# luicalrob/Triangulation-in-Deformable-Scenes

Measured on AMD Instinct MI355X. Metric: LM iterations/sec + ms/iter at 100k corr × 2 views; 1/2/4/8-GPU scaling, higher is better.
Workload: dtype f64

## Files before the change

### triangulation-in-deformable-scenes_amd/csrc/kernels.h

```cpp
#pragma once
#include <hip/hip_runtime.h>

#include <cstdint>
#include <vector>

namespace deftri {

constexpr int64_t kHeavyChunks = 16;

struct DevProblem {
    int32_t P = 0, Q = 0, S = 0, C = 0, R = 0, D = 0, E = 0, NR = 0;
    double *points = nullptr, *scales = nullptr, *tg = nullptr;
    double *points_bak = nullptr, *scales_bak = nullptr, *tg_bak = nullptr;
    float *cam_kb8 = nullptr;
    double *cam_pose = nullptr, *cam_R = nullptr;
    int32_t *rep_point = nullptr, *rep_cam = nullptr;
    double *rep_obs = nullptr, *rep_info = nullptr;
    double huber_delta = 0;
    int32_t *dep_point = nullptr, *dep_scale = nullptr, *dep_cam = nullptr;
    double *dep_meas = nullptr, *dep_info = nullptr;
    int32_t *arap_pts = nullptr, *arap_pair = nullptr, *arap_rot = nullptr;
    double *arap_w = nullptr, *rot = nullptr, *pair_area = nullptr, *pair_info = nullptr;
    double *Jrep = nullptr, *Wrep = nullptr, *Erep = nullptr, *chi_rep = nullptr;
    double *Jdep = nullptr, *Wdep = nullptr, *Edep = nullptr, *chi_dep = nullptr;
    double *Jarap = nullptr, *Warap = nullptr, *Earap = nullptr, *chi_arap = nullptr;
    int64_t jarap_ld = 0;
    double *tg_pre = nullptr;
    const int *gate_lin = nullptr, *gate_trial = nullptr;
    double *lin_part = nullptr;
    int64_t n_arap_sum = 0;
};

struct FrontDev {
    const int32_t *m, *s, *parent, *nchild, *child0, *child1, *direct, *rhs_bnd, *panel_off;
    const int64_t *arena_off, *vec_off, *rows_off, *bmap_off, *inv_off;
    const int32_t *rows, *bmap;
};

struct LevelDev {
    int64_t ea_off[2]; int32_t nea[2];
    struct Step { int64_t diag_off; int32_t ndiag; int64_t trsm_off; int32_t ntrsm; int64_t upd_off; int32_t nupd; int32_t k0, kA, kmax, inner, stream, wait_side; double upd_flops; int32_t ntail, ndiag_tail; };
    std::vector<Step> steps;
    int64_t fwd_off; int32_t nfwd;
    struct SolveStep { int64_t off; int32_t n; };
    std::vector<SolveStep> fsteps, bsteps;
// ... 142 lines not shown
```

### triangulation-in-deformable-scenes_amd/csrc/kernels.hip

```cpp
#include <hip/hip_runtime.h>

#include <algorithm>
#include <atomic>
#include <cstdint>
#include <cstdlib>

#include "device_math.h"
#include "diag_panel.h"
#include "kernels.h"
#include "symbolic.h"
#include "ticket.h"

namespace deftri {
namespace dev {

#define TID (blockIdx.x * blockDim.x + threadIdx.x)

__device__ __forceinline__ void huber_rho(double delta, double e2, double &rho0, double &rho1) {
#pragma clang fp contract(off)
    if (delta <= 0) { rho0 = e2; rho1 = 1.0; return; }
    double dsqr = delta * delta;
    if (e2 <= dsqr) { rho0 = e2; rho1 = 1.0; }
    else { double se = sqrt(e2); rho0 = 2 * se * delta - dsqr; rho1 = delta / se; }
}

__device__ __forceinline__ double lin_rep_edge(int e, int R, const int32_t *__restrict__ rp, const int32_t *__restrict__ rc,
// ... 240 lines not shown
    if (k > 0) {
        const double delta = 1e-9;
        double uu[6] = {0, 0, 0, 0, 0, 0};
        uu[(k - 1) >> 1] = (k & 1) ? delta : -delta;
        X = se3_mul(se3_exp(uu), T);
    }
    double *o = pre + 12 * (int64_t)t;
    quat_to_mat(X.r, o);
    o[9] = X.t[0]; o[10] = X.t[1]; o[11] = X.t[2];
}
__global__ void k_arap_pre(int Q, const double *__restrict__ tg, double *__restrict__ pre, const int *gate) {
    if (gate && !*gate) return;
    arap_pre_one(TID, Q, tg, pre);
}

template <int MODE>
__device__ __forceinline__ double lin_arap_edge(int e, int E_, const int32_t *__restrict__ apts, const int32_t *__restrict__ apair,
                           const int32_t *__restrict__ arot, const double *__restrict__ aw,
                           const double *__restrict__ rot, const double *__restrict__ parea,
                           const double *__restrict__ pinfo, const double *__restrict__ points,
                           const double *__restrict__ tg, const double *__restrict__ tg_pre,
                           double *__restrict__ J, double *__restrict__ W,
                           double *__restrict__ E, double *__restrict__ chi, int want_jac, int analytic,
                           int64_t jld) {
    if (e >= E_) return 0.0;
    const int32_t *v = apts + 4 * (int64_t)e;
    double P[4][3];
#pragma unroll
    for (int k = 0; k < 4; k++) {
        const double *pp = points + 3 * (int64_t)v[k];
        P[k][0] = pp[0]; P[k][1] = pp[1]; P[k][2] = pp[2];
    }
    int q = apair[e];
    SE3 T = se3_load(tg + 7 * q);
    const double *Ri = rot + 9 * (int64_t)arot[2 * (int64_t)e];
    const double *Rj = rot + 9 * (int64_t)arot[2 * (int64_t)e + 1];
    double w = aw[e], om = pinfo[q];
    const AreaDiv area = area_div(parea[q]);
    double err = arap_err(P[0], P[1], P[2], P[3], T, Ri, Rj, w, area);
// ... 25 lines not shown
            Jv[0 + k] = -rv[k] - 2.0 * g[k];
            Jv[3 + k] = qv[k] + rg[k];
            Jv[6 + k] = rv[k] - 2.0 * g[k];
            Jv[9 + k] = -qv[k] + rg[k];
        }
        Jv[12] = 2.0 * (u[1] * g[2] - u[2] * g[1]);
        Jv[13] = 2.0 * (u[2] * g[0] - u[0] * g[2]);
        Jv[14] = 2.0 * (u[0] * g[1] - u[1] * g[0]);
        Jv[15] = -4.0 * g[0]; Jv[16] = -4.0 * g[1]; Jv[17] = -4.0 * g[2];
    } else if (MODE == 2) {
#pragma clang fp contract(off)
        auto jst = [&](int k, double v) {
            if (jld) J[k * jld + e] = v;
            else J[18 * (int64_t)e + k] = v;
        };
        bool negz = false;
#pragma unroll
        for (int a = 0; a < 4; a++)
#pragma unroll
            for (int k = 0; k < 3; k++) negz |= __double_as_longlong(P[a][k]) == (long long)0x8000000000000000ull;
        if (negz) {
            const double delta = 1e-9, scalar = 1.0 / (2 * delta);
            const double *X = tg_pre + 12 * kArapPre * (int64_t)q;
#pragma unroll
            for (int vi = 0; vi < 4; vi++)
#pragma unroll 1
                for (int dd = 0; dd < 3; dd++) {
                    double Pp[4][3], Pm[4][3];
#pragma unroll
                    for (int a = 0; a < 4; a++)
#pragma unroll
                        for (int k = 0; k < 3; k++) {
                            const double d = (a == vi && k == dd) ? delta : 0.0;
                            Pp[a][k] = P[a][k] + d;
                            Pm[a][k] = P[a][k] - d;
                        }
                    const double ep = arap_err_rt(Pp[0], Pp[1], Pp[2], Pp[3], X, X + 9, Ri, Rj, w, area);
                    const double em = arap_err_rt(Pm[0], Pm[1], Pm[2], Pm[3], X, X + 9, Ri, Rj, w, area);
                    jst(3 * vi + dd, scalar * (ep - em));
                }
#pragma unroll 1
            for (int dd = 0; dd < 6; dd++) {
                const double *Xp = X + 12 * (1 + 2 * dd), *Xm = Xp + 12;
                const double ep = arap_err_rt(P[0], P[1], P[2], P[3], Xp, Xp + 9, Ri, Rj, w, area);
                const double em = arap_err_rt(P[0], P[1], P[2], P[3], Xm, Xm + 9, Ri, Rj, w, area);
                jst(12 + dd, scalar * (ep - em));
            }
        } else {
            const double delta = 1e-9, scalar = 1.0 / (2 * delta);
            const double *X = tg_pre + 12 * kArapPre * (int64_t)q;
            double Rg[12];
#pragma unroll
            for (int k = 0; k < 12; k++) Rg[k] = X[k];
            ArapBase bm;
            arap_base(P[0], P[1], P[2], P[3], Rg, Rg + 9, Ri, Rj, area, bm);
            const double fgm = arap_fg(bm.f, bm.g);
#pragma unroll 1
            for (int dd = 0; dd < 6; dd++) {
                const double *Xp = X + 12 * (1 + 2 * dd), *Xm = Xp + 12;
                double dp[3], dm[3];
#pragma unroll
                for (int k = 0; k < 3; k++) {
                    dp[k] = ((arap_mrow(Xp + 3 * k, P[1]) - Xp[9 + k]) - P[0][k]) + ((arap_mrow(Xp + 3 * k, P[3]) - Xp[9 + k]) - P[2][k]);
                    dm[k] = ((arap_mrow(Xm + 3 * k, P[1]) - Xm[9 + k]) - P[0][k]) + ((arap_mrow(Xm + 3 * k, P[3]) - Xm[9 + k]) - P[2][k]);
                }
                jst(12 + dd, scalar * (arap_sum_fg(dp, fgm, w) - arap_sum_fg(dm, fgm, w)));
            }
            auto point = [&](auto VI_, auto DD_) {
                constexpr int VI = decltype(VI_)::value, DD = decltype(DD_)::value;
                const double ep = arap_pert<VI, DD>(bm, P, P[VI][DD] + delta, Rg, Rg + 9, Ri, Rj, w, area);
                const double em = arap_pert<VI, DD>(bm, P, P[VI][DD] - delta, Rg, Rg + 9, Ri, Rj, w, area);
                jst(3 * VI + DD, scalar * (ep - em));
            };
            using std::integral_constant;
            point(integral_constant<int, 0>{}, integral_constant<int, 0>{});
            point(integral_constant<int, 0>{}, integral_constant<int, 1>{});
            point(integral_constant<int, 0>{}, integral_constant<int, 2>{});
            point(integral_constant<int, 1>{}, integral_constant<int, 0>{});
            point(integral_constant<int, 1>{}, integral_constant<int, 1>{});
            point(integral_constant<int, 1>{}, integral_constant<int, 2>{});
            point(integral_constant<int, 2>{}, integral_constant<int, 0>{});
            point(integral_constant<int, 2>{}, integral_constant<int, 1>{});
            point(integral_constant<int, 2>{}, integral_constant<int, 2>{});
            point(integral_constant<int, 3>{}, integral_constant<int, 0>{});
            point(integral_constant<int, 3>{}, integral_constant<int, 1>{});
            point(integral_constant<int, 3>{}, integral_constant<int, 2>{});
        }
    } else {
#pragma clang fp contract(off)
        const double delta = 1e-9, scalar = 1.0 / (2 * delta);
        const double *X = tg_pre + 12 * kArapPre * (int64_t)q;
        double Rg[12];
#pragma unroll
        for (int k = 0; k < 12; k++) Rg[k] = X[k];
#pragma unroll
        for (int vi = 0; vi < 4; vi++)
#pragma unroll 1
            for (int dd = 0; dd < 3; dd++) {
                double Pp[4][3], Pm[4][3];
#pragma unroll
                for (int a = 0; a < 4; a++)
// ... 13 lines not shown
        for (int dd = 0; dd < 6; dd++) {
            const double *Xp = X + 12 * (1 + 2 * dd), *Xm = Xp + 12;
            double ep = arap_err_rt(P[0], P[1], P[2], P[3], Xp, Xp + 9, Ri, Rj, w, area);
            double em = arap_err_rt(P[0], P[1], P[2], P[3], Xm, Xm + 9, Ri, Rj, w, area);
            Jv[12 + dd] = scalar * (ep - em);
        }
    }
    if (MODE != 2) {
        if (jld) {
#pragma unroll
            for (int k = 0; k < 18; k++) J[k * jld + e] = Jv[k];
        } else {
            for (int k = 0; k < 18; k++) J[18 * (int64_t)e + k] = Jv[k];
        }
    }
    W[e] = om;
    E[e] = err;
    return c2;
}

__device__ __forceinline__ double block128_sum(double v) {
    __shared__ double r2[2];
    for (int off = 32; off > 0; off >>= 1) v += __shfl_xor(v, off, 64);
    if ((threadIdx.x & 63) == 0) r2[threadIdx.x >> 6] = v;
    __syncthreads();
    return r2[0] + r2[1];
}

__global__ void k_lin_rep(int R, const int32_t *__restrict__ rp, const int32_t *__restrict__ rc,
                          const double *__restrict__ obs, const double *__restrict__ info, double hdelta,
// ... 11 lines not shown
                          const double *__restrict__ scales, const double *__restrict__ cam_pose,
                          const double *__restrict__ cam_R, double *__restrict__ J, double *__restrict__ W,
                          double *__restrict__ E, double *__restrict__ chi, int want_jac, int analytic, const int *gate) {
    if (gate && !*gate) return;
    lin_dep_edge(TID, D, dpt, dsc, dcam, meas, info, points, scales, cam_pose, cam_R, J, W, E, chi, want_jac, analytic);
}

template <int MODE>
__global__ void __launch_bounds__(128) __attribute__((amdgpu_waves_per_eu(MODE == 2 ? 2 : 1, 8))) k_lin_arap(int E_, const int32_t *__restrict__ apts, const int32_t *__restrict__ apair,
                           const int32_t *__restrict__ arot, const double *__restrict__ aw,
                           const double *__restrict__ rot, const double *__restrict__ parea,
                           const double *__restrict__ pinfo, const double *__restrict__ points,
                           const double *__restrict__ tg, const double *__restrict__ tg_pre,
                           double *__restrict__ J, double *__restrict__ W,
                           double *__restrict__ E, double *__restrict__ chi, int want_jac, int analytic,
                           int64_t jld, const int *gate, double *__restrict__ lpart, int64_t nsum) {
    if (gate && !*gate) return;
    const double c = lin_arap_edge<MODE>(TID, E_, apts, apair, arot, aw, rot, parea, pinfo, points, tg, tg_pre, J, W, E,
                                         lpart ? nullptr : chi, want_jac, analytic, jld);
    if (lpart && (int64_t)blockIdx.x * 128 < nsum) {
        const double v = block128_sum(TID < nsum ? c : 0.0);
        if (threadIdx.x == 0) lpart[blockIdx.x] = v;
    }
}

__global__ void __launch_bounds__(128) k_lin_pts(const DevProblem P, int nbr, int nbd, int want_jac, int analytic) {
    if (P.gate_lin && !*P.gate_lin) return;
    const int b = blockIdx.x, t = threadIdx.x;
    double c = 0.0;
    if (b < nbr)
        c = lin_rep_edge(b * 128 + t, P.R, P.rep_point, P.rep_cam, P.rep_obs, P.rep_info, P.huber_delta, P.points,
                         P.cam_pose, P.cam_R, P.cam_kb8, P.Jrep, P.Wrep, P.Erep, P.lin_part ? nullptr : P.chi_rep,
                         want_jac);
    else if (b < nbr + nbd)
        c = lin_dep_edge((b - nbr) * 128 + t, P.D, P.dep_point, P.dep_scale, P.dep_cam, P.dep_meas, P.dep_info, P.points,
                         P.scales, P.cam_pose, P.cam_R, P.Jdep, P.Wdep, P.Edep, P.lin_part ? nullptr : P.chi_dep,
                         want_jac, analytic);
// ... 1566 lines not shown
    return v;
}

void launch_linearize(const DevProblem &P, hipStream_t st, bool want_jac, bool analytic) {
    const bool pre = want_jac && !analytic && P.E > 0;
    const int nbr = P.R > 0 ? (int)nb(P.R, 128) : 0, nbd = P.D > 0 ? (int)nb(P.D, 128) : 0;
    const int nbp = pre ? (int)nb((int64_t)P.Q * dev::kArapPre, 128) : 0;
    LAUNCH("lin_pts", dev::k_lin_pts, dim3(nbr + nbd + nbp), dim3(128), st, P, nbr, nbd, want_jac ? 1 : 0,
           analytic ? 1 : 0);
    if (P.E > 0)
        LAUNCH("lin_arap", (!want_jac ? dev::k_lin_arap<0> : analytic ? dev::k_lin_arap<1> : arap_j_full() ? dev::k_lin_arap<3> : dev::k_lin_arap<2>),
                           dim3(nb(P.E, 128)), dim3(128), st, P.E, P.arap_pts, P.arap_pair,
                           P.arap_rot, P.arap_w, P.rot, P.pair_area, P.pair_info, P.points, P.tg,
                           pre ? P.tg_pre : nullptr, P.Jarap, P.Warap, P.Earap, P.chi_arap, want_jac ? 1 : 0,
                           analytic ? 1 : 0, P.jarap_ld, P.gate_lin, P.lin_part ? P.lin_part + nbr + nbd : nullptr,
                           P.n_arap_sum);
}

void launch_assemble(const DevProblem &P, const DevPlan &L, hipStream_t st) {
    dev::EdgeJ ej{P.Jrep, P.Wrep, P.Erep, P.Jdep, P.Wdep, P.Edep, P.Jarap, P.Warap, P.Earap};
    if (L.nhchunks > 0)
        LAUNCH("hchunk", dev::k_hchunk, dim3(nb(L.nhchunks, 64)), dim3(64), st, L.nhchunks, L.hcontrib,
                           L.hchunk_begin, L.hchunk_len, ej, L.hpart);
    if (L.nblocks > 0)
        LAUNCH("hfinal", dev::k_hfinal, dim3(nb(L.nblocks, 128)), dim3(128), st, L.nblocks,
                           L.hblk_chunk_begin, L.blk_val_off, L.blk_rows, L.blk_cols, L.hpart, L.hval);
    if (L.nheavy_h > 0) {
        LAUNCH("hfinal_heavy", dev::k_heavy_split<36>, dim3((unsigned)(L.nheavy_h * dev::kHeavySplit)), dim3(256), st,
               L.heavy_h, L.hblk_chunk_begin, L.hpart, L.heavy_scratch);
        LAUNCH("hfinal_heavy", dev::k_heavy_final<36>, dim3((unsigned)L.nheavy_h), dim3(64), st, L.heavy_h,
               L.blk_val_off, L.blk_rows, L.blk_cols, L.heavy_scratch, L.hval);
// ... 321 lines not shown
```

### triangulation-in-deformable-scenes_amd/csrc/spcg.h

```cpp
#pragma once
#include <hip/hip_runtime.h>

#include <cmath>
#include <cstdint>
#include <functional>
#include <string>
#include <vector>

#include "../../include/deftri.h"
#include "kernels.h"

namespace deftri {

constexpr int kSpBlock = 256;
constexpr int kSpRed = 16;
constexpr int kSpPart = 8;
constexpr int kSpLin = 27;
constexpr int kSpSortWindow = 512;
constexpr int kSpWaveSplit = 16;
constexpr int kSpRowSplit = 1;
constexpr int kSpP2Step = 8;
constexpr int kSpGlinGroup = 8;
constexpr int kSpGlinStep = 8;
constexpr int kSpGuessMargin = 1;
constexpr int kSpHeavySplit = 512;
constexpr int kSpUpdRows = 256;
constexpr int kSpHeavyChunk = 128;
constexpr int kSpFuseHeavyMax = 8192;
constexpr int64_t kSpMergeMinDof = 50000;
constexpr int kSpTileUnits = 128;
constexpr int kSpTileLds = 39 * 1024;
constexpr int kSpTilePartsMax = 2048;
constexpr int kSpTileLdsFixed = 2048;
constexpr uint32_t kTmHead = 1u << 24, kTmLast = 1u << 25, kTmSwap = 1u << 26, kTmValid = 1u << 27, kTmCut = 1u << 28;
constexpr uint32_t kTmDrop = 1u << 29, kTmForeign = 1u << 30;
enum { SP_ARAP = 0, SP_DEP = 1 };
enum { kSpRunning = 0, kSpConverged = 1, kSpBreakdown = 2, kSpBadBlock = 3, kSpBudget = 4, kSpTimeout = 5 };

struct SpTransport {
    virtual ~SpTransport() {}
    virtual int allreduce(double *dev, int64_t n, int op, hipStream_t st) = 0;
    struct Op { int peer; bool send; double *buf; int64_t n; };
// ... 78 lines not shown
                            const double *Jr, const double *Wr, const double *Jd, const double *Wd, double lambda,
                            const double *p, double *q, std::string &why);
bool build_sp_plan(const deftri_problem_desc &d, int rank, int nranks, bool fp32_jac, SpPlanHost &out,
                   std::string &err, bool tile = false);
int sp_emulate_product(const deftri_problem_desc &d, const SpPlanHost &H, const double *Ja, const double *Wa,
                       const double *Jr, const double *Wr, const double *Jd, const double *Wd, double lambda,
                       const double *p, double *q, const std::function<int(int, int, double *, int64_t)> &xfer);

struct SpDev {
    int32_t P = 0, Q = 0, S = 0;
    int64_t hd = 0, ndof = 0;
    int32_t row0 = 0, nown = 0;
    int32_t nblk = 0, nrb = 0;
    int32_t include_heavy = 1;
    const int4 *blk = nullptr;
    const int2 *glb = nullptr;
    int32_t nglb = 0;
    const int32_t *hv_blk = nullptr;
    const int64_t *hv_blk_off = nullptr;
    const int32_t *apts = nullptr, *apair = nullptr;
    const double *Ja = nullptr, *Wa = nullptr, *Ea = nullptr;
    const float *Ja32 = nullptr;
    const double *Jr = nullptr, *Wr = nullptr, *Er = nullptr;
    const double *Jd = nullptr, *Wd = nullptr, *Ed = nullptr;
    const int32_t *dsc = nullptr, *drow = nullptr, *dperm = nullptr;
    const int64_t *inc_off = nullptr;
    const int32_t *inc = nullptr, *rep_off = nullptr, *dep_off = nullptr;
    int64_t jld = 0;
    int32_t nwaves = 0, heavy_split = 0;
    int32_t rs = 1, nrb2 = 0;
    int32_t p2u = 8;
    int32_t glu = 8;
// ... 209 lines not shown
```

### triangulation-in-deformable-scenes_amd/csrc/spcg.hip

```cpp
#include <hip/hip_runtime.h>

#include <algorithm>
#include <cstdio>
#include <type_traits>

#include "spcg.h"
#include "ticket.h"
#include "wave.h"

namespace deftri {
namespace sp {

using wv::wave_sum;
using wv::wave_max;

__device__ __forceinline__ double block_sum(double v, double *red4) {
    const int lane = threadIdx.x & 63, w = threadIdx.x >> 6;
    v = wave_sum(v);
    if (lane == 0) red4[w] = v;
    __syncthreads();
    const double s = (red4[0] + red4[1]) + (red4[2] + red4[3]);
    __syncthreads();
    return s;
}
// ... 182 lines not shown
        if (l >= 0) {
#pragma unroll
            for (int k = 0; k < 6; k++) { G.Hv[6 * (int64_t)l + k] = H[k]; G.Dv[6 * (int64_t)l + k] = D[k]; }
            const int64_t o = G.hd + 3 * (int64_t)(G.row0 + l);
#pragma unroll
            for (int a = 0; a < 3; a++) G.b[o + a] = bb[a];
            mx = fmax(fabs(H[0]), fmax(fabs(H[2]), fabs(H[5])));
        }
    }
    mx = wave_max(mx);
    if ((threadIdx.x & 63) == 0) red4[threadIdx.x >> 6] = mx;
    __syncthreads();
    if (threadIdx.x == 0 && lb < max(G.nrb2, 1)) G.mpart[lb] = fmax(fmax(red4[0], red4[1]), fmax(red4[2], red4[3]));
}

__global__ void __launch_bounds__(256) k_sp_glin_blocks(const SpDev G) {
    __shared__ double red[kSpLin][4];
    if (gated_off(G.lgate)) return;
    const int2 gr = G.glb[blockIdx.x];
    const int4 d = G.blk[gr.x];
    const int kind = d.x & 0xff, owned = d.x >> 8;
    const int lane = threadIdx.x & 63, w = threadIdx.x >> 6;
    const int i = d.z + threadIdx.x;
    double *out = G.lpart + (int64_t)kSpLin * gr.x;
    if (kind == SP_ARAP) {
        if (!owned) return;
        double a[kSpLin];
#pragma unroll
        for (int k = 0; k < kSpLin; k++) a[k] = 0.0;
        const int iend = G.blk[gr.x + gr.y - 1].w;
        for (int ii = i; ii < iend; ii += 256) {
            double J[6];
#pragma unroll
            for (int r = 0; r < 6; r++) J[r] = G.Ja[(12 + r) * G.jld + ii];
            const double wv = G.Wa[ii], er = G.Ea[ii];
#pragma unroll
            for (int r = 0; r < 6; r++) {
                const double jr = J[r] * wv;
#pragma unroll
                for (int c = 0; c <= r; c++) a[tri6(r, c)] += jr * J[c];
                a[21 + r] -= J[r] * (wv * er);
            }
        }
        for (int k = threadIdx.x; k < kSpLin * (gr.y - 1); k += 256) out[kSpLin + k] = 0.0;
#pragma unroll
        for (int k = 0; k < kSpLin; k++) {
            const double v = wave_sum(a[k]);
            if (lane == 0) red[k][w] = v;
        }
        __syncthreads();
        if (threadIdx.x < kSpLin) {
            const int k = threadIdx.x;
            out[k] = (red[k][0] + red[k][1]) + (red[k][2] + red[k][3]);
        }
    } else {
        double h = 0.0, bs = 0.0;
        if (i < d.w) {
            const int le = G.dperm[i];
            const double js = G.Jd[4 * (int64_t)le + 3];
            h = G.wss[le];
            bs = -js * (G.Wd[le] * G.Ed[le]);
        }
        h = wave_sum(h);
        bs = wave_sum(bs);
        if (lane == 0) { red[0][w] = h; red[1][w] = bs; }
        __syncthreads();
        if (threadIdx.x < 2) {
            const int k = threadIdx.x;
            out[k] = (red[k][0] + red[k][1]) + (red[k][2] + red[k][3]);
        }
    }
}

__global__ void __launch_bounds__(256) k_sp_glin_heavy(const SpDev G) {
    __shared__ double lds[8][32];
    __shared__ int last;
    if (gated_off(G.lgate)) return;
    const int ch = blockIdx.x, h = G.ch_h[ch];
    const int dim = h < G.Q ? kSpLin : 2;
    const int c = threadIdx.x & 31, g = threadIdx.x >> 5;
    double acc = 0.0;
    if (c < dim) {
        int64_t k = G.ch_lo[ch] + g;
        const int64_t k1 = G.ch_lo[ch + 1];
        for (; k + 7 * 8 < k1; k += 64) {
            double v[8];
#pragma unroll
            for (int u = 0; u < 8; u++) v[u] = G.lpart[(int64_t)kSpLin * G.hv_blk[k + 8 * u] + c];
#pragma unroll
            for (int u = 0; u < 8; u++) acc += v[u];
        }
        for (; k < k1; k += 8) acc += G.lpart[(int64_t)kSpLin * G.hv_blk[k] + c];
    }
    lds[g][c] = acc;
    __syncthreads();
    if ((int)threadIdx.x < dim) {
        double t = 0.0;
#pragma unroll
        for (int gg = 0; gg < 8; gg++) t += lds[gg][threadIdx.x];
        publish(G.chpart + (int64_t)kSpLin * ch + threadIdx.x, t);
    }
    const int c0 = G.hch_off[h], c1 = G.hch_off[h + 1];
    if (threadIdx.x == 0) {
        __atomic_signal_fence(__ATOMIC_SEQ_CST);
        __builtin_amdgcn_s_waitcnt(0);
        __atomic_signal_fence(__ATOMIC_SEQ_CST);
        last = __hip_atomic_fetch_add(G.hcnt + h, 1, __ATOMIC_RELAXED, __HIP_MEMORY_SCOPE_AGENT) == c1 - c0 - 1;
    }
    __syncthreads();
    if (!last) return;
    acc = 0.0;
    if (c < dim)
        for (int j = c0 + g; j < c1; j += 8) acc += fetch(G.chpart + (int64_t)kSpLin * j + c);
    __syncthreads();
    lds[g][c] = acc;
    __syncthreads();
    if ((int)threadIdx.x < dim) {
        double t = 0.0;
#pragma unroll
        for (int gg = 0; gg < 8; gg++) t += lds[gg][threadIdx.x];
        const int q = threadIdx.x;
        if (h < G.Q) {
            if (q < 21) G.hl[21 * (int64_t)h + q] = t;
            else G.b[6 * (int64_t)h + q - 21] = t;
        } else {
            if (q == 0) G.hl[21 * (int64_t)G.Q + (h - G.Q)] = t;
            else G.b[6 * (int64_t)G.Q + (h - G.Q)] = t;
        }
// ... 1619 lines not shown
    else if (G.p2u == 6) SPL("sp_phase2", (sp::k_sp_phase2<JT, MG, 6>), grid, it, G, lambda, pj);
    else SPL("sp_phase2", (sp::k_sp_phase2<JT, MG, 8>), grid, it, G, lambda, pj);
}

void sp_launch_glin(const SpDev &G, bool fp32, hipStream_t st) {
    if (G.glu == 4) {
        if (fp32) SPL("sp_glin_rows", (sp::k_sp_glin_rows<float, 4>), sp::row_grid(G.nrb2), G, G.pj32);
        else SPL("sp_glin_rows", (sp::k_sp_glin_rows<double, 4>), sp::row_grid(G.nrb2), G, G.pj);
    } else if (G.glu == 6) {
        if (fp32) SPL("sp_glin_rows", (sp::k_sp_glin_rows<float, 6>), sp::row_grid(G.nrb2), G, G.pj32);
        else SPL("sp_glin_rows", (sp::k_sp_glin_rows<double, 6>), sp::row_grid(G.nrb2), G, G.pj);
    } else {
        if (fp32) SPL("sp_glin_rows", (sp::k_sp_glin_rows<float, 8>), sp::row_grid(G.nrb2), G, G.pj32);
        else SPL("sp_glin_rows", (sp::k_sp_glin_rows<double, 8>), sp::row_grid(G.nrb2), G, G.pj);
    }
    if (G.nblk > 0) SPL("sp_glin_blocks", sp::k_sp_glin_blocks, G.nglb, G);
    if (G.nch > 0) SPL("sp_glin_heavy", sp::k_sp_glin_heavy, G.nch, G);
}

void sp_launch_maxdiag(const SpDev &G, double *out, hipStream_t st) {
    SPL("sp_maxdiag", sp::k_sp_maxdiag, 1, G, out, 0);
}

void sp_launch_maxdiag_heavy(const SpDev &G, double *out, hipStream_t st) {
    SPL("sp_maxdiag", sp::k_sp_maxdiag, 1, G, out, 1);
}

void sp_launch_cvt_j(const double *J, float *J32, int64_t n, hipStream_t st, const int *gate) {
    if (n > 0) SPL("sp_cvt_j", sp::k_sp_cvt_j, nblk(n, 256), J, J32, n, gate);
}

// ... 126 lines not shown
```

### triangulation-in-deformable-scenes_amd/csrc/spcg_solver.cpp

```cpp
#include <hip/hip_runtime.h>

#include <algorithm>
#include <atomic>
#include <chrono>
#include <thread>
#include <cmath>
#include <cstdio>
#include <cstdlib>
#include <cstring>
#include <limits>

#include "host_threads.h"
#include "spcg.h"
#include "ticket.h"

namespace deftri {

void sp_launch_maxdiag_heavy(const SpDev &G, double *out, hipStream_t st);

namespace {
constexpr int kSpMaxIt = 4096;
constexpr int kSpDefaultIt = 1000;
constexpr int kSpRedParts = 512;
constexpr int kSpRecDoubles = 8;
hipError_t stream_wait(hipStream_t st) {
    static const bool block = std::getenv("DEFTRI_SYNC_BLOCK") != nullptr;
// ... 243 lines not shown
    pts.clear(); pts.shrink_to_fit();
    apts.clear(); apts.shrink_to_fit();

    G.P = NP; G.Q = Q; G.S = S;
    G.hd = H.hd;
    G.ndof = H.hd + 3 * (int64_t)NP;
    G.row0 = H.lo; G.nown = nown;
    G.nblk = (int32_t)(H.blk.size() / 4);
    G.nrb = (nown + kSpBlock - 1) / kSpBlock;
    G.include_heavy = rank_ == 0 ? 1 : 0;
    int32_t *blk, *hvb, *dperm, *inc, *roff, *doff;
    int64_t *hvbo, *inco;
    PUT(blk, H.blk); PUT(hvb, H.hv_blk); PUT(hvbo, H.hv_blk_off); PUT(dperm, H.dperm);
    PUT(inc, H.inc); PUT(inco, H.inc_off); PUT(roff, H.rep_off); PUT(doff, H.dep_off);
    G.blk = reinterpret_cast<const int4 *>(blk);
    {
        const int gmax = kSpGlinGroup;
        std::vector<int32_t> gl;
        const int32_t nb = (int32_t)(H.blk.size() / 4);
        for (int32_t b = 0; b < nb;) {
            const int32_t *d0 = &H.blk[4 * (size_t)b];
            const bool arap_owned = (d0[0] & 0xff) == SP_ARAP && (d0[0] >> 8) != 0;
            int32_t n = 1;
            while (arap_owned && n < gmax && b + n < nb) {
                const int32_t *dn = &H.blk[4 * (size_t)(b + n)], *dp = dn - 4;
                if (dn[0] != d0[0] || dn[1] != d0[1] || dn[2] != dp[3]) break;
                n++;
            }
            gl.push_back(b);
            gl.push_back(n);
            b += n;
        }
        int32_t *glb;
        PUT(glb, gl);
        G.glb = reinterpret_cast<const int2 *>(glb);
        G.nglb = (int32_t)(gl.size() / 2);
    }
    G.hv_blk = hvb; G.hv_blk_off = hvbo; G.dperm = dperm;
    G.inc = inc; G.inc_off = inco; G.rep_off = roff; G.dep_off = doff;
    G.apts = P.arap_pts; G.apair = P.arap_pair;
    G.Ja = P.Jarap; G.Wa = P.Warap; G.Ea = P.Earap;
    G.pinfo = P.pair_info;
    G.Jr = P.Jrep; G.Wr = P.Wrep; G.Er = P.Erep;
    G.Jd = P.Jdep; G.Wd = P.Wdep; G.Ed = P.Edep;
    G.dsc = P.dep_scale; G.drow = P.dep_point;
    G.jld = P.jarap_ld;
    if (fp32_jac) { float *j32; ALLOC(j32, 18 * G.jld); G.Ja32 = j32; }
    G.nwaves = (int32_t)(H.woff.size() - 1);
    G.nslots = H.woff.back();
    G.heavy_split = H.max_heavy_blocks > kSpHeavySplit ? 1 : 0;
    {
// ... 39 lines not shown
        int64_t *wo;
        uint8_t *ws;
        PUT(rm, H.rowmap); PUT(wo, H.woff); PUT(pm, H.pmap); PUT(pi, H.pidx); PUT(ws, H.wsplit);
        G.rowmap = rm; G.woff = wo; G.pmap = pm; G.pidx = pi; G.wsplit = ws;
        if (H.tile && (G.merged || G.sd)) { G.pj = nullptr; G.pj32 = nullptr; }
        else if (fp32_jac) { ALLOC(G.pj32, 3 * 64 * G.nslots); }
        else { ALLOC(G.pj, 3 * 64 * G.nslots); }
        H.pmap.clear(); H.pmap.shrink_to_fit();
        H.pidx.clear(); H.pidx.shrink_to_fit();
    }
    ALLOC(G.Hv, 6 * (int64_t)nown); ALLOC(G.Dv, 6 * (int64_t)nown); ALLOC(G.Mv, 6 * (int64_t)nown);
    ALLOC(G.cdep, 3 * (int64_t)nd); ALLOC(G.wss, nd);
    ALLOC(G.hl, 21 * (int64_t)Q + S + G.ndof);
    G.b = G.hl + 21 * (int64_t)Q + S;
    ALLOC(G.Mh, 36 * (int64_t)Q + S);
    ALLOC(G.lpart, (int64_t)kSpLin * G.nblk); ALLOC(G.mpart, std::max(std::max(G.nrb2, 8 * ((G.nrb + 7) / 8)), 1));
    ALLOC(G.r, G.ndof); ALLOC(G.q, G.ndof); ALLOC(G.x, G.ndof);
    int64_t nrecv = 0;
    for (const auto &v : H.recv_rows) nrecv += (int64_t)v.size();
    const int64_t zp_n = G.ndof + (G.sd ? 3 * nrecv : 0);
    double *zp;
    ALLOC(zp, 2 * zp_n);
    G.zp = reinterpret_cast<double2 *>(zp);
    if (H.tile && (G.merged || G.sd)) {
        G.tile = 1;
        G.ntile = H.ntile;
        G.tile_lds = H.tile_lds;
        G.tile_segmax = H.tile_segmax;
        G.t_grid = 8 * ((H.ntile + 7) / 8) + 1;
        int32_t *tt, *trs, *th, *txo, *txd, *tch;
        uint32_t *tm;
// ... 48 lines not shown
        G.tparts = (G.sd || G.t_grid > kSpTilePartsMax) ? 0 : 1;
    }
    ALLOC(G.s, nloc); ALLOC(G.part, (int64_t)kSpPart * std::max(G.nblk, G.t_grid)); ALLOC(G.rpart, std::max(G.nrb2, 1));
    ALLOC(G.upart, 2 * (int64_t)(G.nrb + 1)); ALLOC(G.hbuf, 1 + H.hd);
    ALLOC(G.rec, kSpRecDoubles + (int64_t)kSpRed * (kSpMaxIt + 2));
    ALLOC(G.ph, std::max<int64_t>(H.hd, 1));
    G.m1n = G.tile ? G.t_grid : sp_merged_grid1(G);
    ALLOC(G.m1part, std::max(G.m1n, sp_merged_grid1(G)));
    ALLOC(G.m2part, 2 * (int64_t)std::max(sp_merged_grid2(G), G.m_nh + 8 * ((G.nrb + 7) / 8))); ALLOC(G.gsum, 32);
    ALLOC(G.cnt, 64);
    SPOK(hipMemset(G.cnt, 0, 64 * sizeof(int)));
    {
        std::vector<int32_t> chh, hcho(Q + S + 1, 0);
        std::vector<int64_t> chlo;
        for (int32_t h = 0; h < Q + S; h++) {
            const int64_t k0 = H.hv_blk_off[h], k1 = H.hv_blk_off[h + 1];
            int64_t k = k0;
            do {
                chh.push_back(h);
                chlo.push_back(k);
                k = std::min<int64_t>(k + kSpHeavyChunk, k1);
            } while (k < k1);
            hcho[h + 1] = (int32_t)chh.size();
        }
        chlo.push_back(H.hv_blk_off.empty() ? 0 : H.hv_blk_off.back());
        G.nch = (int32_t)chh.size();
        int32_t *d_chh, *d_hcho;
        int64_t *d_chlo;
        PUT(d_chh, chh); PUT(d_hcho, hcho); PUT(d_chlo, chlo);
        G.ch_h = d_chh; G.hch_off = d_hcho; G.ch_lo = d_chlo;
        ALLOC(G.chpart, (int64_t)kSpLin * std::max(G.nch, 1));
        ALLOC(G.hcnt, std::max(Q + S, 1));
        SPOK(hipMemset(G.hcnt, 0, sizeof(int) * (size_t)std::max(Q + S, 1)));
    }
    G.red = G.rec + kSpRecDoubles;
    SPOK(hipMemset(G.x, 0, sizeof(double) * (size_t)G.ndof));
    SPOK(hipMemset(G.zp, 0, sizeof(double) * 2 * (size_t)zp_n));
    SPOK(hipMemset(G.rec, 0, sizeof(double) * (size_t)(kSpRecDoubles + kSpRed * (kSpMaxIt + 2))));
    ALLOC(d_scal, 8); ALLOC(d_part, kMaxSumJobs * kSpRedParts); ALLOC(d_flag, 1); ALLOC(d_sumcnt, 16);
    {
// ... 896 lines not shown
```

### triangulation-in-deformable-scenes_amd/csrc/wave.h

```cpp
#pragma once
#include <hip/hip_runtime.h>

namespace deftri {
namespace wv {

template <int CTRL>
__device__ __forceinline__ double dpp(double v) {
    int2 p = __builtin_bit_cast(int2, v);
    p.x = __builtin_amdgcn_update_dpp(0, p.x, CTRL, 0xf, 0xf, true);
    p.y = __builtin_amdgcn_update_dpp(0, p.y, CTRL, 0xf, 0xf, true);
    return __builtin_bit_cast(double, p);
}
__device__ __forceinline__ void swap16(double v, double &a, double &b) {
    const int2 p = __builtin_bit_cast(int2, v);
    const auto lo = __builtin_amdgcn_permlane16_swap((unsigned)p.x, (unsigned)p.x, false, false);
    const auto hi = __builtin_amdgcn_permlane16_swap((unsigned)p.y, (unsigned)p.y, false, false);
    a = __builtin_bit_cast(double, make_int2((int)lo[0], (int)hi[0]));
    b = __builtin_bit_cast(double, make_int2((int)lo[1], (int)hi[1]));
}
__device__ __forceinline__ void swap32(double v, double &a, double &b) {
    const int2 p = __builtin_bit_cast(int2, v);
    const auto lo = __builtin_amdgcn_permlane32_swap((unsigned)p.x, (unsigned)p.x, false, false);
    const auto hi = __builtin_amdgcn_permlane32_swap((unsigned)p.y, (unsigned)p.y, false, false);
    a = __builtin_bit_cast(double, make_int2((int)lo[0], (int)hi[0]));
    b = __builtin_bit_cast(double, make_int2((int)lo[1], (int)hi[1]));
}
__device__ __forceinline__ double wave_sum(double v) {
    v += dpp<0xB1>(v);
    v += dpp<0x4E>(v);
    v += dpp<0x141>(v);
    v += dpp<0x140>(v);
    double a, b;
    swap16(v, a, b);
    v = a + b;
    swap32(v, a, b);
    return a + b;
}

__device__ __forceinline__ double wave_max(double v) {
    v = fmax(v, dpp<0xB1>(v));
    v = fmax(v, dpp<0x4E>(v));
    v = fmax(v, dpp<0x141>(v));
    v = fmax(v, dpp<0x140>(v));
    double a, b;
    swap16(v, a, b);
    v = fmax(a, b);
    swap32(v, a, b);
    return fmax(a, b);
}

}
}
```

Before: 1727.

## Fuse ARAP heavy-row partial sums into linearize kernel via wave-level multi-reduction

Removes the separate sp_glin_blocks kernel. Each wave of the ARAP linearize kernel now reduces the per-pair 6x6 Hessian and gradient contributions directly, using a new transpose-style multi-value wave reduction, and writes one slot per distinct pair per wave. The heavy-row gather kernel reads these slots through a host-built pair-sorted index. The depth-scale path now reads the depth edges directly in contiguous chunks, with a host check that they are contiguous. This saves a kernel launch and a reread of the Jacobian, W and E arrays, at the cost of more register pressure and more reduction work inside the linearize kernel.

New measurement: 1745, median of 4. 1.01x the previous value.

```diff
diff --git a/triangulation-in-deformable-scenes_amd/csrc/arap_heavy_slots.h b/triangulation-in-deformable-scenes_amd/csrc/arap_heavy_slots.h
--- /dev/null
+++ b/triangulation-in-deformable-scenes_amd/csrc/arap_heavy_slots.h
@@ -0,0 +1,25 @@
+#pragma once
+#include <cstdint>
+#include <vector>
+
+namespace deftri {
+
+constexpr int kArapHeavy = 27;
+
+inline void arap_heavy_slots(const int32_t *apair, int64_t n_owned, std::vector<int32_t> &wslot,
+                             std::vector<int32_t> &slot_pair) {
+    wslot.clear();
+    slot_pair.clear();
+    for (int64_t e0 = 0; e0 < n_owned; e0 += 64) {
+        const size_t first = slot_pair.size();
+        wslot.push_back((int32_t)first);
+        const int64_t e1 = e0 + 64 < n_owned ? e0 + 64 : n_owned;
+        for (int64_t e = e0; e < e1; e++) {
+            bool seen = false;
+            for (size_t k = first; k < slot_pair.size() && !seen; k++) seen = slot_pair[k] == apair[e];
+            if (!seen) slot_pair.push_back(apair[e]);
+        }
+    }
+}
+
+}
diff --git a/triangulation-in-deformable-scenes_amd/csrc/kernels.h b/triangulation-in-deformable-scenes_amd/csrc/kernels.h
--- a/triangulation-in-deformable-scenes_amd/csrc/kernels.h
+++ b/triangulation-in-deformable-scenes_amd/csrc/kernels.h
@@ -29,6 +29,8 @@
     const int *gate_lin = nullptr, *gate_trial = nullptr;
     double *lin_part = nullptr;
     int64_t n_arap_sum = 0;
+    double *heavy_part = nullptr;
+    const int32_t *heavy_wslot = nullptr;
 };
 
 struct FrontDev {
diff --git a/triangulation-in-deformable-scenes_amd/csrc/kernels.hip b/triangulation-in-deformable-scenes_amd/csrc/kernels.hip
--- a/triangulation-in-deformable-scenes_amd/csrc/kernels.hip
+++ b/triangulation-in-deformable-scenes_amd/csrc/kernels.hip
@@ -5,11 +5,13 @@
 #include <cstdint>
 #include <cstdlib>
 
+#include "arap_heavy_slots.h"
 #include "device_math.h"
 #include "diag_panel.h"
 #include "kernels.h"
 #include "symbolic.h"
 #include "ticket.h"
+#include "wave.h"
 
 namespace deftri {
 namespace dev {
@@ -280,6 +282,8 @@
     arap_pre_one(TID, Q, tg, pre);
 }
 
+struct ArapHeavyIn { double t[6], err, om; };
+
 template <int MODE>
 __device__ __forceinline__ double lin_arap_edge(int e, int E_, const int32_t *__restrict__ apts, const int32_t *__restrict__ apair,
                            const int32_t *__restrict__ arot, const double *__restrict__ aw,
@@ -288,7 +292,8 @@
                            const double *__restrict__ tg, const double *__restrict__ tg_pre,
                            double *__restrict__ J, double *__restrict__ W,
                            double *__restrict__ E, double *__restrict__ chi, int want_jac, int analytic,
-                           int64_t jld) {
+                           int64_t jld, ArapHeavyIn *hv = nullptr) {
+    if (hv) *hv = ArapHeavyIn{{0, 0, 0, 0, 0, 0}, 0, 0};
     if (e >= E_) return 0.0;
     const int32_t *v = apts + 4 * (int64_t)e;
     double P[4][3];
@@ -344,6 +349,11 @@
             if (jld) J[k * jld + e] = v;
             else J[18 * (int64_t)e + k] = v;
         };
+        auto hst = [&](int dd, double v) {
+            if (!hv) return;
+#pragma unroll
+            for (int k = 0; k < 6; k++) hv->t[k] = dd == k ? v : hv->t[k];
+        };
         bool negz = false;
 #pragma unroll
         for (int a = 0; a < 4; a++)
@@ -374,7 +384,9 @@
                 const double *Xp = X + 12 * (1 + 2 * dd), *Xm = Xp + 12;
                 const double ep = arap_err_rt(P[0], P[1], P[2], P[3], Xp, Xp + 9, Ri, Rj, w, area);
                 const double em = arap_err_rt(P[0], P[1], P[2], P[3], Xm, Xm + 9, Ri, Rj, w, area);
-                jst(12 + dd, scalar * (ep - em));
+                const double jv = scalar * (ep - em);
+                jst(12 + dd, jv);
+                hst(dd, jv);
             }
         } else {
             const double delta = 1e-9, scalar = 1.0 / (2 * delta);
@@ -384,18 +396,6 @@
             for (int k = 0; k < 12; k++) Rg[k] = X[k];
             ArapBase bm;
             arap_base(P[0], P[1], P[2], P[3], Rg, Rg + 9, Ri, Rj, area, bm);
-            const double fgm = arap_fg(bm.f, bm.g);
-#pragma unroll 1
-            for (int dd = 0; dd < 6; dd++) {
-                const double *Xp = X + 12 * (1 + 2 * dd), *Xm = Xp + 12;
-                double dp[3], dm[3];
-#pragma unroll
-                for (int k = 0; k < 3; k++) {
-                    dp[k] = ((arap_mrow(Xp + 3 * k, P[1]) - Xp[9 + k]) - P[0][k]) + ((arap_mrow(Xp + 3 * k, P[3]) - Xp[9 + k]) - P[2][k]);
-                    dm[k] = ((arap_mrow(Xm + 3 * k, P[1]) - Xm[9 + k]) - P[0][k]) + ((arap_mrow(Xm + 3 * k, P[3]) - Xm[9 + k]) - P[2][k]);
-                }
-                jst(12 + dd, scalar * (arap_sum_fg(dp, fgm, w) - arap_sum_fg(dm, fgm, w)));
-            }
             auto point = [&](auto VI_, auto DD_) {
                 constexpr int VI = decltype(VI_)::value, DD = decltype(DD_)::value;
                 const double ep = arap_pert<VI, DD>(bm, P, P[VI][DD] + delta, Rg, Rg + 9, Ri, Rj, w, area);
@@ -415,6 +415,20 @@
             point(integral_constant<int, 3>{}, integral_constant<int, 0>{});
             point(integral_constant<int, 3>{}, integral_constant<int, 1>{});
             point(integral_constant<int, 3>{}, integral_constant<int, 2>{});
+            const double fgm = arap_fg(bm.f, bm.g);
+#pragma unroll 1
+            for (int dd = 0; dd < 6; dd++) {
+                const double *Xp = X + 12 * (1 + 2 * dd), *Xm = Xp + 12;
+                double dp[3], dm[3];
+#pragma unroll
+                for (int k = 0; k < 3; k++) {
+                    dp[k] = ((arap_mrow(Xp + 3 * k, P[1]) - Xp[9 + k]) - P[0][k]) + ((arap_mrow(Xp + 3 * k, P[3]) - Xp[9 + k]) - P[2][k]);
+                    dm[k] = ((arap_mrow(Xm + 3 * k, P[1]) - Xm[9 + k]) - P[0][k]) + ((arap_mrow(Xm + 3 * k, P[3]) - Xm[9 + k]) - P[2][k]);
+                }
+                const double jv = scalar * (arap_sum_fg(dp, fgm, w) - arap_sum_fg(dm, fgm, w));
+                jst(12 + dd, jv);
+                hst(dd, jv);
+            }
         }
     } else {
 #pragma clang fp contract(off)
@@ -458,6 +472,13 @@
             for (int k = 0; k < 18; k++) J[18 * (int64_t)e + k] = Jv[k];
         }
     }
+    if (hv) {
+        if (MODE != 2)
+#pragma unroll
+            for (int k = 0; k < 6; k++) hv->t[k] = Jv[12 + k];
+        hv->err = err;
+        hv->om = om;
+    }
     W[e] = om;
     E[e] = err;
     return c2;
@@ -499,13 +520,42 @@
                            const double *__restrict__ tg, const double *__restrict__ tg_pre,
                            double *__restrict__ J, double *__restrict__ W,
                            double *__restrict__ E, double *__restrict__ chi, int want_jac, int analytic,
-                           int64_t jld, const int *gate, double *__restrict__ lpart, int64_t nsum) {
+                           int64_t jld, const int *gate, double *__restrict__ lpart, int64_t nsum,
+                           double *__restrict__ hpart, const int32_t *__restrict__ hslot) {
     if (gate && !*gate) return;
+    ArapHeavyIn hv;
     const double c = lin_arap_edge<MODE>(TID, E_, apts, apair, arot, aw, rot, parea, pinfo, points, tg, tg_pre, J, W, E,
-                                         lpart ? nullptr : chi, want_jac, analytic, jld);
+                                         lpart ? nullptr : chi, want_jac, analytic, jld, MODE != 0 ? &hv : nullptr);
     if (lpart && (int64_t)blockIdx.x * 128 < nsum) {
         const double v = block128_sum(TID < nsum ? c : 0.0);
         if (threadIdx.x == 0) lpart[blockIdx.x] = v;
+    }
+    if constexpr (MODE != 0) {
+        const int64_t wave = (int64_t)blockIdx.x * 2 + (threadIdx.x >> 6);
+        if (hpart && wave * 64 < nsum) {
+            const int64_t e = TID;
+            const int lane = threadIdx.x & 63;
+            const int q = e < nsum ? apair[e] : -1;
+            const int k = wv::wave_sums_index(lane);
+            double *out = hpart + kArapHeavy * (int64_t)hslot[wave];
+            unsigned long long todo = __ballot(q >= 0);
+            while (todo) {
+                const int qq = __shfl(q, __ffsll(todo) - 1);
+                const bool in = q == qq;
+                double a[kArapHeavy];
+#pragma unroll
+                for (int r = 0; r < 6; r++) {
+                    const double jr = in ? hv.t[r] * hv.om : 0.0;
+#pragma unroll
+                    for (int cc = 0; cc <= r; cc++) a[r * (r + 1) / 2 + cc] = in ? jr * hv.t[cc] : 0.0;
+                    a[21 + r] = in ? -(hv.t[r] * (hv.om * hv.err)) : 0.0;
+                }
+                const double v = wv::wave_sums(a, lane);
+                if (!(lane & 1) && k < kArapHeavy) out[k] = v;
+                todo &= ~__ballot(in);
+                out += kArapHeavy;
+            }
+        }
     }
 }
 
@@ -2102,7 +2152,7 @@
                            P.arap_rot, P.arap_w, P.rot, P.pair_area, P.pair_info, P.points, P.tg,
                            pre ? P.tg_pre : nullptr, P.Jarap, P.Warap, P.Earap, P.chi_arap, want_jac ? 1 : 0,
                            analytic ? 1 : 0, P.jarap_ld, P.gate_lin, P.lin_part ? P.lin_part + nbr + nbd : nullptr,
-                           P.n_arap_sum);
+                           P.n_arap_sum, want_jac ? P.heavy_part : nullptr, P.heavy_wslot);
 }
 
 void launch_assemble(const DevProblem &P, const DevPlan &L, hipStream_t st) {
diff --git a/triangulation-in-deformable-scenes_amd/csrc/spcg.h b/triangulation-in-deformable-scenes_amd/csrc/spcg.h
--- a/triangulation-in-deformable-scenes_amd/csrc/spcg.h
+++ b/triangulation-in-deformable-scenes_amd/csrc/spcg.h
@@ -20,12 +20,12 @@
 constexpr int kSpWaveSplit = 16;
 constexpr int kSpRowSplit = 1;
 constexpr int kSpP2Step = 8;
-constexpr int kSpGlinGroup = 8;
 constexpr int kSpGlinStep = 8;
 constexpr int kSpGuessMargin = 1;
 constexpr int kSpHeavySplit = 512;
 constexpr int kSpUpdRows = 256;
 constexpr int kSpHeavyChunk = 128;
+constexpr int kSpHeavyDepthChunk = 1024;
 constexpr int kSpFuseHeavyMax = 8192;
 constexpr int64_t kSpMergeMinDof = 50000;
 constexpr int kSpTileUnits = 128;
@@ -134,8 +134,7 @@
     int32_t nblk = 0, nrb = 0;
     int32_t include_heavy = 1;
     const int4 *blk = nullptr;
-    const int2 *glb = nullptr;
-    int32_t nglb = 0;
+    const int32_t *hv_lin = nullptr;
     const int32_t *hv_blk = nullptr;
     const int64_t *hv_blk_off = nullptr;
     const int32_t *apts = nullptr, *apair = nullptr;
diff --git a/triangulation-in-deformable-scenes_amd/csrc/spcg.hip b/triangulation-in-deformable-scenes_amd/csrc/spcg.hip
--- a/triangulation-in-deformable-scenes_amd/csrc/spcg.hip
+++ b/triangulation-in-deformable-scenes_amd/csrc/spcg.hip
@@ -220,91 +220,68 @@
     if (threadIdx.x == 0 && lb < max(G.nrb2, 1)) G.mpart[lb] = fmax(fmax(red4[0], red4[1]), fmax(red4[2], red4[3]));
 }
 
-__global__ void __launch_bounds__(256) k_sp_glin_blocks(const SpDev G) {
-    __shared__ double red[kSpLin][4];
-    if (gated_off(G.lgate)) return;
-    const int2 gr = G.glb[blockIdx.x];
-    const int4 d = G.blk[gr.x];
-    const int kind = d.x & 0xff, owned = d.x >> 8;
-    const int lane = threadIdx.x & 63, w = threadIdx.x >> 6;
-    const int i = d.z + threadIdx.x;
-    double *out = G.lpart + (int64_t)kSpLin * gr.x;
-    if (kind == SP_ARAP) {
-        if (!owned) return;
-        double a[kSpLin];
-#pragma unroll
-        for (int k = 0; k < kSpLin; k++) a[k] = 0.0;
-        const int iend = G.blk[gr.x + gr.y - 1].w;
-        for (int ii = i; ii < iend; ii += 256) {
-            double J[6];
-#pragma unroll
-            for (int r = 0; r < 6; r++) J[r] = G.Ja[(12 + r) * G.jld + ii];
-            const double wv = G.Wa[ii], er = G.Ea[ii];
-#pragma unroll
-            for (int r = 0; r < 6; r++) {
-                const double jr = J[r] * wv;
-#pragma unroll
-                for (int c = 0; c <= r; c++) a[tri6(r, c)] += jr * J[c];
-                a[21 + r] -= J[r] * (wv * er);
-            }
-        }
-        for (int k = threadIdx.x; k < kSpLin * (gr.y - 1); k += 256) out[kSpLin + k] = 0.0;
-#pragma unroll
-        for (int k = 0; k < kSpLin; k++) {
-            const double v = wave_sum(a[k]);
-            if (lane == 0) red[k][w] = v;
-        }
-        __syncthreads();
-        if (threadIdx.x < kSpLin) {
-            const int k = threadIdx.x;
-            out[k] = (red[k][0] + red[k][1]) + (red[k][2] + red[k][3]);
-        }
-    } else {
-        double h = 0.0, bs = 0.0;
-        if (i < d.w) {
-            const int le = G.dperm[i];
-            const double js = G.Jd[4 * (int64_t)le + 3];
-            h = G.wss[le];
-            bs = -js * (G.Wd[le] * G.Ed[le]);
-        }
-        h = wave_sum(h);
-        bs = wave_sum(bs);
-        if (lane == 0) { red[0][w] = h; red[1][w] = bs; }
-        __syncthreads();
-        if (threadIdx.x < 2) {
-            const int k = threadIdx.x;
-            out[k] = (red[k][0] + red[k][1]) + (red[k][2] + red[k][3]);
-        }
-    }
-}
-
 __global__ void __launch_bounds__(256) k_sp_glin_heavy(const SpDev G) {
     __shared__ double lds[8][32];
+    __shared__ double red4[4];
     __shared__ int last;
     if (gated_off(G.lgate)) return;
     const int ch = blockIdx.x, h = G.ch_h[ch];
     const int dim = h < G.Q ? kSpLin : 2;
     const int c = threadIdx.x & 31, g = threadIdx.x >> 5;
     double acc = 0.0;
-    if (c < dim) {
-        int64_t k = G.ch_lo[ch] + g;
-        const int64_t k1 = G.ch_lo[ch + 1];
-        for (; k + 7 * 8 < k1; k += 64) {
-            double v[8];
-#pragma unroll
-            for (int u = 0; u < 8; u++) v[u] = G.lpart[(int64_t)kSpLin * G.hv_blk[k + 8 * u] + c];
-#pragma unroll
-            for (int u = 0; u < 8; u++) acc += v[u];
-        }
-        for (; k < k1; k += 8) acc += G.lpart[(int64_t)kSpLin * G.hv_blk[k] + c];
-    }
-    lds[g][c] = acc;
-    __syncthreads();
-    if ((int)threadIdx.x < dim) {
-        double t = 0.0;
-#pragma unroll
-        for (int gg = 0; gg < 8; gg++) t += lds[gg][threadIdx.x];
-        publish(G.chpart + (int64_t)kSpLin * ch + threadIdx.x, t);
+    if (h >= G.Q) {
+        constexpr int U = kSpHeavyDepthChunk / 256;
+        const int64_t k0 = G.ch_lo[2 * ch] + threadIdx.x, k1 = G.ch_lo[2 * ch + 1];
+        const int32_t *__restrict__ dperm = G.dperm;
+        const double *__restrict__ Jd = G.Jd, *__restrict__ Wd = G.Wd, *__restrict__ Ed = G.Ed, *__restrict__ wss = G.wss;
+        double hs = 0.0, bs = 0.0;
+        if (G.ch_lo[2 * ch] < k1) {
+            int le[U];
+            double js[U], ws[U], wd[U], ed[U];
+#pragma unroll
+            for (int u = 0; u < U; u++) le[u] = dperm[min(k0 + 256 * u, k1 - 1)];
+#pragma unroll
+            for (int u = 0; u < U; u++) {
+                const int64_t j = le[u];
+                js[u] = Jd[4 * j + 3];
+                ws[u] = wss[j];
+                wd[u] = Wd[j];
+                ed[u] = Ed[j];
+            }
+#pragma unroll
+            for (int u = 0; u < U; u++) {
+                const bool in = k0 + 256 * u < k1;
+                hs += in ? ws[u] : 0.0;
+                bs += in ? -js[u] * (wd[u] * ed[u]) : 0.0;
+            }
+        }
+        hs = block_sum(hs, red4);
+        bs = block_sum(bs, red4);
+        if (threadIdx.x < 2) publish(G.chpart + (int64_t)kSpLin * ch + threadIdx.x, threadIdx.x == 0 ? hs : bs);
+    } else {
+        const int64_t k1 = G.ch_lo[2 * ch + 1];
+        if (c < dim && G.ch_lo[2 * ch] < k1) {
+            const int32_t *__restrict__ hv_lin = G.hv_lin;
+            const double *__restrict__ lpart = G.lpart;
+            for (int64_t k = G.ch_lo[2 * ch] + g; k < k1; k += 16 * 8) {
+                int32_t s[16];
+                double v[16];
+#pragma unroll
+                for (int u = 0; u < 16; u++) s[u] = hv_lin[min(k + 8 * u, k1 - 1)];
+#pragma unroll
+                for (int u = 0; u < 16; u++) v[u] = lpart[(int64_t)kSpLin * s[u] + c];
+#pragma unroll
+                for (int u = 0; u < 16; u++) acc += k + 8 * u < k1 ? v[u] : 0.0;
+            }
+        }
+        lds[g][c] = acc;
+        __syncthreads();
+        if ((int)threadIdx.x < dim) {
+            double t = 0.0;
+#pragma unroll
+            for (int gg = 0; gg < 8; gg++) t += lds[gg][threadIdx.x];
+            publish(G.chpart + (int64_t)kSpLin * ch + threadIdx.x, t);
+        }
     }
     const int c0 = G.hch_off[h], c1 = G.hch_off[h + 1];
     if (threadIdx.x == 0) {
@@ -317,7 +294,13 @@
     if (!last) return;
     acc = 0.0;
     if (c < dim)
-        for (int j = c0 + g; j < c1; j += 8) acc += fetch(G.chpart + (int64_t)kSpLin * j + c);
+        for (int j = c0 + g; j < c1; j += 8 * 8) {
+            double v[8];
+#pragma unroll
+            for (int u = 0; u < 8; u++) v[u] = fetch(G.chpart + (int64_t)kSpLin * min(j + 8 * u, c1 - 1) + c);
+#pragma unroll
+            for (int u = 0; u < 8; u++) acc += j + 8 * u < c1 ? v[u] : 0.0;
+        }
     __syncthreads();
     lds[g][c] = acc;
     __syncthreads();
@@ -1967,7 +1950,6 @@
         if (fp32) SPL("sp_glin_rows", (sp::k_sp_glin_rows<float, 8>), sp::row_grid(G.nrb2), G, G.pj32);
         else SPL("sp_glin_rows", (sp::k_sp_glin_rows<double, 8>), sp::row_grid(G.nrb2), G, G.pj);
     }
-    if (G.nblk > 0) SPL("sp_glin_blocks", sp::k_sp_glin_blocks, G.nglb, G);
     if (G.nch > 0) SPL("sp_glin_heavy", sp::k_sp_glin_heavy, G.nch, G);
 }
 
diff --git a/triangulation-in-deformable-scenes_amd/csrc/spcg_solver.cpp b/triangulation-in-deformable-scenes_amd/csrc/spcg_solver.cpp
--- a/triangulation-in-deformable-scenes_amd/csrc/spcg_solver.cpp
+++ b/triangulation-in-deformable-scenes_amd/csrc/spcg_solver.cpp
@@ -10,6 +10,7 @@
 #include <cstring>
 #include <limits>
 
+#include "arap_heavy_slots.h"
 #include "host_threads.h"
 #include "spcg.h"
 #include "ticket.h"
@@ -283,27 +284,35 @@
     PUT(blk, H.blk); PUT(hvb, H.hv_blk); PUT(hvbo, H.hv_blk_off); PUT(dperm, H.dperm);
     PUT(inc, H.inc); PUT(inco, H.inc_off); PUT(roff, H.rep_off); PUT(doff, H.dep_off);
     G.blk = reinterpret_cast<const int4 *>(blk);
+    std::vector<int64_t> hv_lin_off(Q + 1, 0), dep_lo(S, 0), dep_hi(S, 0);
+    int64_t n_lin_part = 0;
     {
-        const int gmax = kSpGlinGroup;
-        std::vector<int32_t> gl;
-        const int32_t nb = (int32_t)(H.blk.size() / 4);
-        for (int32_t b = 0; b < nb;) {
-            const int32_t *d0 = &H.blk[4 * (size_t)b];
-            const bool arap_owned = (d0[0] & 0xff) == SP_ARAP && (d0[0] >> 8) != 0;
-            int32_t n = 1;
-            while (arap_owned && n < gmax && b + n < nb) {
-                const int32_t *dn = &H.blk[4 * (size_t)(b + n)], *dp = dn - 4;
-                if (dn[0] != d0[0] || dn[1] != d0[1] || dn[2] != dp[3]) break;
-                n++;
-            }
-            gl.push_back(b);
-            gl.push_back(n);
-            b += n;
-        }
-        int32_t *glb;
-        PUT(glb, gl);
-        G.glb = reinterpret_cast<const int2 *>(glb);
-        G.nglb = (int32_t)(gl.size() / 2);
+        static_assert(kArapHeavy == kSpLin, "k_lin_arap's partials are k_sp_glin_heavy's");
+        std::vector<int32_t> wslot, slot_pair, hv_lin;
+        arap_heavy_slots(apair.data(), H.n_arap_owned, wslot, slot_pair);
+        for (int32_t q : slot_pair) hv_lin_off[q + 1]++;
+        for (int32_t q = 0; q < Q; q++) hv_lin_off[q + 1] += hv_lin_off[q];
+        hv_lin.resize(slot_pair.size());
+        std::vector<int64_t> pos(hv_lin_off.begin(), hv_lin_off.end() - 1);
+        for (size_t k = 0; k < slot_pair.size(); k++) hv_lin[pos[slot_pair[k]]++] = (int32_t)k;
+        n_lin_part = (int64_t)slot_pair.size();
+        std::vector<int64_t> dep_n(S, 0);
+        const int64_t nb = (int64_t)(H.blk.size() / 4);
+        for (int64_t b = 0; b < nb; b++) {
+            const int32_t *d4 = &H.blk[4 * (size_t)b];
+            if ((d4[0] & 0xff) != SP_DEP) continue;
+            const int32_t s = d4[1];
+            if (dep_n[s] == 0) { dep_lo[s] = d4[2]; dep_hi[s] = d4[3]; }
+            dep_lo[s] = std::min<int64_t>(dep_lo[s], d4[2]);
+            dep_hi[s] = std::max<int64_t>(dep_hi[s], d4[3]);
+            dep_n[s] += d4[3] - d4[2];
+        }
+        for (int32_t s = 0; s < S; s++)
+            if (dep_n[s] != dep_hi[s] - dep_lo[s]) return fail(DEFTRI_E_ARG, "plan: a scale's depth edges are not contiguous");
+        int32_t *d_wslot, *d_hvl;
+        PUT(d_wslot, wslot); PUT(d_hvl, hv_lin);
+        G.hv_lin = d_hvl;
+        P.heavy_wslot = d_wslot;
     }
     G.hv_blk = hvb; G.hv_blk_off = hvbo; G.dperm = dperm;
     G.inc = inc; G.inc_off = inco; G.rep_off = roff; G.dep_off = doff;
@@ -373,7 +382,9 @@
     ALLOC(G.hl, 21 * (int64_t)Q + S + G.ndof);
     G.b = G.hl + 21 * (int64_t)Q + S;
     ALLOC(G.Mh, 36 * (int64_t)Q + S);
-    ALLOC(G.lpart, (int64_t)kSpLin * G.nblk); ALLOC(G.mpart, std::max(std::max(G.nrb2, 8 * ((G.nrb + 7) / 8)), 1));
+    ALLOC(G.lpart, (int64_t)kSpLin * n_lin_part);
+    P.heavy_part = G.lpart;
+    ALLOC(G.mpart, std::max(std::max(G.nrb2, 8 * ((G.nrb + 7) / 8)), 1));
     ALLOC(G.r, G.ndof); ALLOC(G.q, G.ndof); ALLOC(G.x, G.ndof);
     int64_t nrecv = 0;
     for (const auto &v : H.recv_rows) nrecv += (int64_t)v.size();
@@ -452,16 +463,18 @@
         std::vector<int32_t> chh, hcho(Q + S + 1, 0);
         std::vector<int64_t> chlo;
         for (int32_t h = 0; h < Q + S; h++) {
-            const int64_t k0 = H.hv_blk_off[h], k1 = H.hv_blk_off[h + 1];
+            const bool pair = h < Q;
+            const int64_t k0 = pair ? hv_lin_off[h] : dep_lo[h - Q], k1 = pair ? hv_lin_off[h + 1] : dep_hi[h - Q];
+            const int64_t step = pair ? kSpHeavyChunk : kSpHeavyDepthChunk;
             int64_t k = k0;
             do {
                 chh.push_back(h);
                 chlo.push_back(k);
-                k = std::min<int64_t>(k + kSpHeavyChunk, k1);
+                k = std::min<int64_t>(k + step, k1);
+                chlo.push_back(k);
             } while (k < k1);
             hcho[h + 1] = (int32_t)chh.size();
         }
-        chlo.push_back(H.hv_blk_off.empty() ? 0 : H.hv_blk_off.back());
         G.nch = (int32_t)chh.size();
         int32_t *d_chh, *d_hcho;
         int64_t *d_chlo;
diff --git a/triangulation-in-deformable-scenes_amd/csrc/wave.h b/triangulation-in-deformable-scenes_amd/csrc/wave.h
--- a/triangulation-in-deformable-scenes_amd/csrc/wave.h
+++ b/triangulation-in-deformable-scenes_amd/csrc/wave.h
@@ -37,6 +37,60 @@
     return a + b;
 }
 
+__device__ __forceinline__ void swap32(double x, double y, double &a, double &b) {
+    const int2 p = __builtin_bit_cast(int2, x), q = __builtin_bit_cast(int2, y);
+    const auto lo = __builtin_amdgcn_permlane32_swap((unsigned)p.x, (unsigned)q.x, false, false);
+    const auto hi = __builtin_amdgcn_permlane32_swap((unsigned)p.y, (unsigned)q.y, false, false);
+    a = __builtin_bit_cast(double, make_int2((int)lo[0], (int)hi[0]));
+    b = __builtin_bit_cast(double, make_int2((int)lo[1], (int)hi[1]));
+}
+__device__ __forceinline__ void swap16(double x, double y, double &a, double &b) {
+    const int2 p = __builtin_bit_cast(int2, x), q = __builtin_bit_cast(int2, y);
+    const auto lo = __builtin_amdgcn_permlane16_swap((unsigned)p.x, (unsigned)q.x, false, false);
+    const auto hi = __builtin_amdgcn_permlane16_swap((unsigned)p.y, (unsigned)q.y, false, false);
+    a = __builtin_bit_cast(double, make_int2((int)lo[0], (int)hi[0]));
+    b = __builtin_bit_cast(double, make_int2((int)lo[1], (int)hi[1]));
+}
+__device__ __forceinline__ int wave_sums_index(int lane) {
+    return ((lane >> 5) & 1) | ((lane >> 4) & 1) << 1 | ((lane >> 3) & 1) << 2 | ((lane >> 2) & 1) << 3 | ((lane >> 1) & 1) << 4;
+}
+template <int N>
+__device__ __forceinline__ double wave_sums(const double (&in)[N], int lane) {
+    static_assert(N >= 1 && N <= 32, "one value per lane pair at most");
+    constexpr int n1 = (N + 1) / 2, n2 = (n1 + 1) / 2, n3 = (n2 + 1) / 2, n4 = (n3 + 1) / 2;
+    double v[N];
+#pragma unroll
+    for (int i = 0; i < N; i++) v[i] = in[i];
+#pragma unroll
+    for (int i = 0; i < n1; i++) {
+        double a, b;
+        swap32(v[2 * i], 2 * i + 1 < N ? v[2 * i + 1] : 0.0, a, b);
+        v[i] = a + b;
+    }
+#pragma unroll
+    for (int i = 0; i < n2; i++) {
+        double a, b;
+        swap16(v[2 * i], 2 * i + 1 < n1 ? v[2 * i + 1] : 0.0, a, b);
+        v[i] = a + b;
+    }
+    const bool h3 = lane & 8, h2 = lane & 4, h1 = lane & 2;
+#pragma unroll
+    for (int i = 0; i < n3; i++) {
+        const double x = v[2 * i], y = 2 * i + 1 < n2 ? v[2 * i + 1] : 0.0;
+        v[i] = (h3 ? y : x) + dpp<0x140>(h3 ? x : y);
+    }
+#pragma unroll
+    for (int i = 0; i < n4; i++) {
+        const double x = v[2 * i], y = 2 * i + 1 < n3 ? v[2 * i + 1] : 0.0;
+        v[i] = (h2 ? y : x) + dpp<0x141>(h2 ? x : y);
+    }
+    {
+        const double x = v[0], y = 1 < n4 ? v[1] : 0.0;
+        v[0] = (h1 ? y : x) + dpp<0x4E>(h1 ? x : y);
+    }
+    return v[0] + dpp<0xB1>(v[0]);
+}
+
 __device__ __forceinline__ double wave_max(double v) {
     v = fmax(v, dpp<0xB1>(v));
     v = fmax(v, dpp<0x4E>(v));
```
